# ricklisz/AnatoMask

Hardware: AMD Instinct MI355X
Metric: pretrain volumes/sec @128^3 patch mask=0.6 (higher is better)
Workload: dtype bf16; 1 GPU; STUNet-B AnatoMask step, 128^3 patch, mask_ratio 0.6, bf16 storage/MFMA + fp32 master; per_gpu_batch=16, global_batch=16, parallelism=dp1, step=teacher fwd + sampler + student fwd + loss + bwd + clip + AdamW + EMA

## Files before the change

### anatomask_amd/csrc/stream_ops.hip

```cpp
#include <mutex>
#include <type_traits>
#include "common.h"
#include "../../include/anatomask_hip.h"

namespace {

constexpr int NREP = 8;

struct Geo {
  int B, D, H, W, C;
  int vpw;
  unsigned mW, mH, mD;
  MaskView mask;
  __device__ __forceinline__ bool active(long v) const {
    if (!mask.m) return true;
    const unsigned u = (unsigned)v;
    const unsigned t1 = __umulhi(u, mW); const int w = u - t1 * W;
    const unsigned t2 = __umulhi(t1, mH); const int h = t1 - t2 * H;
    const unsigned b = __umulhi(t2, mD); const int d = t2 - b * D;
    return mask.active((int)b, d, h, w);
  }
  __device__ __forceinline__ void decode(long v, int& b, int& d, int& h, int& w) const {
    const unsigned u = (unsigned)v;
    const unsigned t1 = __umulhi(u, mW); w = u - t1 * W;
// ... 1223 lines not shown
#pragma unroll
      for (int i = 0; i < EPC; ++i) a1[i] += red[(vl * wk.cpv + threadIdx.x) * 8 + i];
#pragma unroll
    for (int i = 0; i < EPC; ++i) atomicAdd(&ar[threadIdx.x * EPC + i], a1[i]);
  }
  if (threadIdx.x == 0) atomicAdd(&ar[C], (double)redb[0] + (double)redb[1] + (double)redb[2] + (double)redb[3]);
  if (!last_workgroup(fin.ticket)) return;
  if (threadIdx.x == 0) {
    double t = 0.0;
    for (int r = 0; r < NREP; ++r) t += __longlong_as_double(atomicExch((unsigned long long*)&acc[(size_t)r * (C + 1) + C], 0ull));
    s0sh = t;
    fin.db[0] += (float)t;
  }
  __syncthreads();
  const double S0 = s0sh;
  for (int c = threadIdx.x; c < C; c += blockDim.x) {
    double S1 = 0.0;
    for (int r = 0; r < NREP; ++r) S1 += __longlong_as_double(atomicExch((unsigned long long*)&acc[(size_t)r * (C + 1) + c], 0ull));
    const double wc = fin.w[c], rs = fin.rstd[c];
    const double b1 = wc * S0, b2 = rs * wc * S1;
    const float gr = fin.gamma[c] * fin.rstd[c];
    fin.k0w[c] = gr * fin.w[c]; fin.k1[c] = gr * (float)(b1 / fin.n); fin.k2[c] = gr * (float)(b2 / fin.n);
    fin.dgamma[c] += (float)b2;
    fin.dbeta[c] += (float)b1;
    fin.dw[c] += (float)((double)fin.scale[c] * S1 + (double)fin.beta[c] * S0);
  }
  if (threadIdx.x == 0) atomicExch(fin.ticket, 0u);
}

template <typename T>
__global__ __launch_bounds__(256) void proj_norm_bwd_apply_kernel(const T* __restrict__ x, const float* __restrict__ drec, long nvox, int C,
                                                                  int vpw, const float* __restrict__ mean, const float* __restrict__ rstd,
                                                                  const float* __restrict__ k0w, const float* __restrict__ k1,
                                                                  const float* __restrict__ k2, T* __restrict__ dx) {
  constexpr int EPC = TT<T>::EPC;
  Walk<T> wk(C);
  if (!wk.live) return;
  float mu[EPC], c0[EPC], c1[EPC], c2[EPC];
#pragma unroll
  for (int i = 0; i < EPC; ++i) {
    const int c = wk.cl * EPC + i;
    mu[i] = mean[c]; c0[i] = k0w[c]; c1[i] = k1[c]; c2[i] = k2[c] * rstd[c];
  }
  const long v0 = (long)blockIdx.x * vpw, v1 = min(v0 + (long)vpw, nvox);
  for (long v = v0 + wk.vl; v < v1; v += wk.vpp) {
    const float d = drec[v];
    const size_t off = (size_t)v * C + wk.cl * EPC;
    float f[EPC], r[EPC];
    chunk_to_f<T>(*(const u32x4*)(x + off), f);
#pragma unroll
    for (int i = 0; i < EPC; ++i) r[i] = c0[i] * d - c1[i] - c2[i] * (f[i] - mu[i]);
    *(u32x4*)(dx + off) = f_to_chunk<T>(r);
  }
}

template <typename T>
__global__ __launch_bounds__(256) void proj_bwd_kernel(const T* __restrict__ x, const float* __restrict__ drec, long nvox, int C, int vpw,
                                                       const float* __restrict__ w, T* __restrict__ dx, float* __restrict__ dw,
                                                       float* __restrict__ db, float* __restrict__ det_ws) {
  constexpr int EPC = TT<T>::EPC;
  __shared__ float red[256 * 8];
  __shared__ float redb[4];
  Walk<T> wk(C);
  float sw[EPC], wv[EPC], sb = 0.f;
#pragma unroll
  for (int i = 0; i < EPC; ++i) { sw[i] = 0.f; wv[i] = wk.live ? w[wk.cl * EPC + i] : 0.f; }
  const long v0 = (long)blockIdx.x * vpw, v1 = min(v0 + (long)vpw, nvox);
  if (wk.live)
    for (long v = v0 + wk.vl; v < v1; v += wk.vpp) {
      const float d = drec[v];
      const size_t off = (size_t)v * C + wk.cl * EPC;
      float f[EPC], o[EPC];
      chunk_to_f<T>(*(const u32x4*)(x + off), f);
#pragma unroll
      for (int i = 0; i < EPC; ++i) { sw[i] += d * f[i]; o[i] = d * wv[i]; }
      *(u32x4*)(dx + off) = f_to_chunk<T>(o);
      if (wk.cl == 0) sb += d;
    }
#pragma unroll
  for (int i = 0; i < EPC; ++i) red[threadIdx.x * 8 + i] = sw[i];
  sb = warp_sum(sb);
  if ((threadIdx.x & 63) == 0) redb[threadIdx.x >> 6] = sb;
  __syncthreads();
  if (threadIdx.x < wk.cpv) {
    float a1[EPC];
#pragma unroll
// ... 590 lines not shown
}

int am_proj_fwd(int dtype, const void* x, long nvox, int C, const float* w, const float* b, const float* pre_scale, const float* pre_shift,
                float* rec, void* stream) {
  if (!am_row_ok(dtype, C, F32_MAX_C_256)) return -1;
  if ((pre_scale == nullptr) != (pre_shift == nullptr)) return -1;
  hipStream_t st = (hipStream_t)stream;
  const int nb = (int)((nvox + 255) / 256);
  am_by_dtype(dtype, [&](auto t) {
    using T = typename decltype(t)::type;
    AM_LAUNCH(proj_fwd_kernel<T>, dim3(nb), dim3(256), 0, st, (const T*)x, nvox, C, w, b, pre_scale, pre_shift, rec);
  });
  AM_CHECK_LAUNCH();
  return 0;
}

int am_proj_norm_bwd(int dtype, const void* x, const float* drec, long nvox, int C, const float* w, const float* gamma, const float* beta,
                     const float* mean, const float* rstd, const float* scale, double* workspace, float* coef, void* dx,
                     float* dgamma_accum, float* dbeta_accum, float* dw_accum, float* db_accum, void* stream) {
  if (!am_row_ok(dtype, C, F32_MAX_C_256)) return -1;
  if (!x || !drec || !w || !gamma || !beta || !mean || !rstd || !scale || !workspace || !coef || !dx || !dgamma_accum || !dbeta_accum ||
      !dw_accum || !db_accum || nvox <= 0) return -1;
  hipStream_t st = (hipStream_t)stream;
  ProjNormFin fin{(unsigned*)(workspace + (size_t)NREP * (C + 1)), (double)nvox, gamma, beta, rstd, scale, w,
                  coef, coef + C, coef + 2 * C, dgamma_accum, dbeta_accum, dw_accum, db_accum};
  const int vr = pick_vpw(nvox, C, dtype, true), va = pick_vpw(nvox, C, dtype, false);
  am_by_dtype(dtype, [&](auto t) {
    using T = typename decltype(t)::type;
    AM_LAUNCH(proj_norm_bwd_reduce_kernel<T>, dim3(nblk(nvox, vr)), dim3(256), 0, st, (const T*)x, drec, nvox, C, vr, mean, workspace, fin);
  });
  AM_CHECK_LAUNCH();
  am_by_dtype(dtype, [&](auto t) {
    using T = typename decltype(t)::type;
    AM_LAUNCH(proj_norm_bwd_apply_kernel<T>, dim3(nblk(nvox, va)), dim3(256), 0, st, (const T*)x, drec, nvox, C, va, mean, rstd, coef, coef + C, coef + 2 * C, (T*)dx);
  });
  AM_CHECK_LAUNCH();
  return 0;
}

int am_proj_bwd(int dtype, const void* x, const float* drec, long nvox, int C, const float* w, void* dx, float* dw_accum,
                float* db_accum, float* det_workspace, long det_workspace_floats, void* stream) {
  if (!am_row_ok(dtype, C, F32_MAX_C_256)) return -1;
  hipStream_t st = (hipStream_t)stream;
  const int vpw = pick_vpw(nvox, C, dtype, true);
  const int nb = nblk(nvox, vpw);
  if (det_workspace && det_workspace_floats < (long)nb * (C + 1)) return -6;
  am_by_dtype(dtype, [&](auto t) {
    using T = typename decltype(t)::type;
    AM_LAUNCH(proj_bwd_kernel<T>, dim3(nb), dim3(256), 0, st, (const T*)x, drec, nvox, C, vpw, w, (T*)dx, dw_accum, db_accum, det_workspace);
  });
  AM_CHECK_LAUNCH();
  if (det_workspace) {
    AM_LAUNCH(rows_fold_kernel, dim3((C + 1 + 255) / 256), dim3(256), 0, st, det_workspace, nb, C + 1, C, dw_accum, db_accum);
    AM_CHECK_LAUNCH();
  }
  return 0;
}

int am_partials_reduce(const float* partials, int rows, int C, double* sums, float* sum_accum, void* stream) {
  hipStream_t st = (hipStream_t)stream;
  if ((256 % C == 0 || C % 256 == 0) && rows >= 64) {
    const int rstep = C <= 256 ? 256 / C : 1;
    int nb = rows / (rstep * 16); nb = nb < 1 ? 1 : (nb > 256 ? 256 : nb);
    const int rpb = ((rows + nb - 1) / nb + rstep - 1) / rstep * rstep;
    nb = (rows + rpb - 1) / rpb;
    if (sums) AM_HIP(hipMemsetAsync(sums, 0, sizeof(double) * 2 * C, st));
    AM_LAUNCH(partials_reduce2_kernel, dim3(nb), dim3(256), 0, st, partials, rows, C, rpb, sums, sum_accum);
// ... 83 lines not shown
```

### anatomask_amd/engine.py

```python
from __future__ import annotations

from dataclasses import dataclass, field
from typing import Dict, List, Optional, Sequence, Tuple

import torch

from . import ops
from .ops import ACT_LRELU, ACT_NONE, ACT_RELU6, CONV_DGRAD, CONV_FWD, CONVT_DGRAD, CONVT_FWD, MaskInfo, NormStats

ENC = "sparse_encoder.sp_cnn.conv_blocks_context"
DEC = "dense_decoder.dec"


@dataclass
class Spec:
    dims: Sequence[int]
    depth: Sequence[int]
    width: int
    input_size: Tuple[int, int, int]
    in_ch: int = 1
    out_ch: int = 1
    downsample: int = 16
    n_stage: int = 5
    sync_bn: bool = False
# ... 261 lines not shown
    x = None
    for s in range(spec.n_stage):
        sp = spec.stage_spatial(s)
        if tape is not None and recompute:
            tape.enc_in.append(x)
        for b in range(spec.depth[s]):
            x, rec_ = _enc_block(W, pk, inp, mask, counts, sp, s, b, x, keep=tape is not None)
            if tape is not None and not recompute:
                tape.enc.append(rec_)
        feats.append(x)
    return feats


def densify_forward(spec: Spec, W, pk: PackCache, feats, mask: MaskInfo, counts, tape: Optional[Tape] = None) -> List[torch.Tensor]:
    n_dec = len(spec.dec_chs) - 1
    to_dec = []
    for i in range(n_dec):
        f = feats[4 - i]
        st = _sparse_norm(f, mask, i, counts, W[f"densify_norms.{i}.weight"], W[f"densify_norms.{i}.bias"], 1e-6)
        d = ops.norm_apply(f, st, ACT_NONE, mask, i, fill=W[f"mask_tokens.{i}"].view(-1))
        pw = f"densify_projs.{i}.weight"
        if pw in W:
            k = W[pw].shape[-1]
            pr = ops.conv3d(CONV_FWD, d, pk.get(W, pw, False, False), W[f"densify_projs.{i}.bias"], tuple(d.shape[1:4]), k, 1)
        else:
            pr = d
        to_dec.append(pr)
        if tape is not None:
            tape.dens.append({"i": i, "f": f, "st": st, "d": d, "k": W[pw].shape[-1] if pw in W else 0})
    return to_dec


HEAD_STENCIL = True


def decoder_forward(spec: Spec, W, pk: PackCache, to_dec, train: bool, tape: Optional[Tape] = None, recompute: bool = False,
                    needed_patches: Optional[MaskInfo] = None, fuse_eval: Optional[bool] = None, l2_of: Optional[tuple] = None) -> torch.Tensor:
    n_dec = len(spec.dec_chs) - 1
    if fuse_eval is None:
        fuse_eval = tape is None
    x = to_dec[0]
    head = bool(train and FUSED_HEAD and _sync_world(spec.sync_bn) <= 1 and not spec.dec_inorm)
    st_head = None
    for i in range(n_dec):
        nxt = to_dec[i + 1] if i + 1 < n_dec else None
        last = i == n_dec - 1
        o, rec_ = _dec_block(W, pk, i, x, nxt, train, fuse_eval=fuse_eval,
                             out_skip=needed_patches if (last and tape is None and not train) else None, sync=spec.sync_bn,
                             head=head and last, inorm=spec.dec_inorm,
                             stencil_tail=bool(HEAD_STENCIL and last and tape is None and not train and fuse_eval and not spec.dec_inorm))
        if rec_ is not None and rec_.get("stencil"):
            q = f"{DEC}.{i}"
            weff, beff = ops.head_fold(W[f"{q}.conv.3.weight"], rec_["st2"].scale, rec_["st2"].shift, W["dense_decoder.proj.weight"].view(-1),
                                       W["dense_decoder.proj.bias"])
            B_, D_, H_, W_ = o.shape[:4]
            patches = needed_patches
            if patches is None:
                patches = MaskInfo(torch.ones(B_, D_ // 16, H_ // 16, W_ // 16, device=o.device, dtype=torch.uint8), n_active=B_ * (D_ // 16) * (H_ // 16) * (W_ // 16))
            if l2_of is not None:
                ops.head_stencil(o, weff, beff, patches, inp=l2_of[0], l2=l2_of[1])
                return None
            rec = torch.empty(B_, D_, H_, W_, device=o.device, dtype=torch.float32)
            ops.head_stencil(o, weff, beff, patches, rec=rec)
            return rec
        if head and last:
            st_head = rec_["st2"]
        if tape is not None:
            tape.dec.append({"q": rec_["q"], "xin": x, "nxt": nxt, "head": head and last} if recompute else rec_)
        x = o
    rec = ops.proj_fwd(x, W["dense_decoder.proj.weight"].view(-1), W["dense_decoder.proj.bias"], pre=st_head)
    if tape is not None:
        tape.last = x
    return rec


def forward(spec: Spec, W: Dict[str, torch.Tensor], pk: PackCache, inp: torch.Tensor, mask: MaskInfo, train: bool,
            tape: Optional[Tape] = None, want_feats: bool = False, encoder_only: bool = False, recompute: bool = False,
            want_to_dec0: bool = False, needed_patches: Optional[MaskInfo] = None, l2_out: Optional[torch.Tensor] = None):
    counts = _counts(mask, range(5))
    if tape is not None:
        tape.counts = counts
        tape.recompute = recompute
    feats = encoder_forward(spec, W, pk, inp, mask, counts, tape, recompute)
    if encoder_only:
        return feats
    to_dec = densify_forward(spec, W, pk, feats, mask, counts, tape)
    rec = decoder_forward(spec, W, pk, to_dec, train, tape, recompute, needed_patches, l2_of=(inp, l2_out) if l2_out is not None else None)
    if want_to_dec0:
        return rec, to_dec[0]
    return (rec, feats) if want_feats else rec


FUSED_HEAD = True
_SIDE: Dict[int, "torch.cuda.Stream"] = {}
_SIDE_KEEP: Dict[int, List[torch.Tensor]] = {}
_USE_SIDE = True


def _dev_index(dev) -> int:
    return dev.index if dev.index is not None else torch.cuda.current_device()


def _side_stream(dev) -> "torch.cuda.Stream":
    i = _dev_index(dev)
    if i not in _SIDE:
        _SIDE[i] = torch.cuda.Stream(device=dev)
    return _SIDE[i]


def _on_side(dev, tensors, fn):
    if not _USE_SIDE:
        return fn()
    s2 = _side_stream(dev)
    ev = torch.cuda.Event()
    ev.record()
    s2.wait_event(ev)
    _SIDE_KEEP.setdefault(_dev_index(dev), []).extend(tensors)
    with torch.cuda.stream(s2):
        fn()


def _join_side(dev):
    i = _dev_index(dev)
    if _USE_SIDE and i in _SIDE:
        ev = torch.cuda.Event()
        ev.record(_SIDE[i])
        torch.cuda.current_stream(dev).wait_event(ev)
    _SIDE_KEEP.pop(i, None)


def _wgrad_into(pk: PackCache, G, name, mode, x, dy, k, stride, transposed=False, **masks):
    def run():
        dwp = ops.conv3d_wgrad(mode, x, dy, k, stride, f32_split=pk.f32_split, deterministic=pk.deterministic, **masks)
        ops.unpack_grad(dwp, G[name], transposed, accumulate=True)
    _on_side(x.device, (x, dy), run)


def _dec_block_backward(W, G, pk: PackCache, t: dict, g: Optional[torch.Tensor], drec: Optional[torch.Tensor], bias_sum_into: Optional[torch.Tensor]):
    q = t["q"]
    if t.get("inorm"):
        so = tuple(t["r"].shape[1:4])
        dc2 = _instance_norm_backward(g, t["c2"], t["st2"], ACT_NONE)
        dr = ops.conv3d(CONV_DGRAD, dc2, pk.get(W, f"{q}.conv.3.weight", False, True), None, so, 3, 1)
        _wgrad_into(pk, G, f"{q}.conv.3.weight", CONV_FWD, t["r"], dc2, 3, 1)
        dc1 = _instance_norm_backward(dr, t["c1"], t["st1"], ACT_RELU6)
    elif t.get("head"):
        dc2 = ops.proj_norm_bwd(t["c2"], t["st2"], drec, W["dense_decoder.proj.weight"].view(-1), W[f"{q}.conv.4.weight"],
                                W[f"{q}.conv.4.bias"], G[f"{q}.conv.4.weight"], G[f"{q}.conv.4.bias"],
                                G["dense_decoder.proj.weight"].view(-1), G["dense_decoder.proj.bias"])
    else:
        dc2 = ops.norm_backward(g, None, t["c2"], t["st2"], W[f"{q}.conv.4.weight"], ACT_NONE, None, 0,
                                G[f"{q}.conv.4.weight"], G[f"{q}.conv.4.bias"])
    if not t.get("inorm"):
        so = tuple(t["r"].shape[1:4])
        fuse = ops.FUSED_NORM_BWD_REDUCE and dc2.dtype == torch.bfloat16 and t["st1"].sync_world <= 1 and dc2.shape[-1] >= 128
        dr = ops.conv3d(CONV_DGRAD, dc2, pk.get(W, f"{q}.conv.3.weight", False, True), None, so, 3, 1,
                        norm_bwd=(t["c1"], t["st1"], ACT_RELU6) if fuse else None)
        dr, red1 = dr if fuse else (dr, None)
        _wgrad_into(pk, G, f"{q}.conv.3.weight", CONV_FWD, t["r"], dc2, 3, 1)
        dc1 = ops.norm_backward(dr, None, t["c1"], t["st1"], W[f"{q}.conv.1.weight"], ACT_RELU6, None, 0,
                                G[f"{q}.conv.1.weight"], G[f"{q}.conv.1.bias"], reduced=red1)
    du, ptu = ops.conv3d(CONV_DGRAD, dc1, pk.get(W, f"{q}.conv.0.weight", False, True), None, so, 3, 1, want_partials=True, partials_sum_only=True)
    ptu.finalize(None, sum_accum=G[f"{q}.up_sample.bias"])
    _wgrad_into(pk, G, f"{q}.conv.0.weight", CONV_FWD, t["u"], dc1, 3, 1)
    si = tuple(t["xin"].shape[1:4])
    gin = ops.conv3d(CONVT_DGRAD, du, pk.get(W, f"{q}.up_sample.weight", True, True), None, si, 4, 2, want_partials=bias_sum_into is not None)
    if bias_sum_into is not None:
        gin, ptg = gin
        ptg.finalize(None, sum_accum=bias_sum_into)
    _wgrad_into(pk, G, f"{q}.up_sample.weight", CONVT_FWD, t["xin"], du, 4, 2, transposed=True)
    return gin


def decoder_backward(spec: Spec, W, G, pk: PackCache, tape: Tape, drec: torch.Tensor, after_group=None) -> List[Optional[torch.Tensor]]:
    n_dec = len(spec.dec_chs) - 1
    fused_head = bool(tape.dec[n_dec - 1].get("head"))
    g = None
    if not fused_head:
# ... 175 lines not shown
```

### anatomask_amd/hip.py

```python
import ctypes as C
import os
import re

_HERE = os.path.dirname(os.path.abspath(__file__))
LIB_PATH = os.path.join(_HERE, "libanatomask_hip.so")
HEADER = os.path.join(os.path.dirname(_HERE), "include", "anatomask_hip.h")

DT_F32, DT_BF16, DT_F32S = 0, 1, 2
CONV_FWD, CONV_DGRAD, CONVT_FWD, CONVT_DGRAD = 0, 1, 2, 3
ACT_NONE, ACT_LRELU, ACT_RELU6 = 0, 1, 2

_CT = {"int": C.c_int, "long": C.c_long, "float": C.c_float, "double": C.c_double}


def declared_functions(header: str = HEADER):
    txt = open(header).read()
    txt = re.sub(r"/\*.*?\*/", " ", txt, flags=re.S)
    out = {}
    for m in re.finditer(r"\bint\s+(am_\w+)\s*\(([^;]*?)\)\s*;", txt, flags=re.S):
        name, args = m.group(1), m.group(2).strip()
        types = []
        if args and args != "void":
            for a in args.split(","):
                a = " ".join(a.split())
                if "*" in a:
                    types.append(C.c_void_p)
                else:
                    types.append(_CT[a.replace("const ", "").split(" ")[0]])
        out[name] = types
    return out


class HipLib:
    ANSWERS = ("am_head_stencil_supported", "am_conv3d_wgrad_uses_k3", "am_conv3d_uses_k3", "am_conv3d_prenorm_supported", "am_version")

    def __init__(self, path: str = LIB_PATH):
        import torch
        if not os.path.exists(path):
            raise RuntimeError(f"{path} not built: run `python -m anatomask_amd.build` (no fallback path exists)")
        if os.path.abspath(path) == LIB_PATH:
            from . import build as _b
            sp = _b.stamp_path(path)
            have = open(sp).read().strip() if os.path.exists(sp) else None
            if have != _b.source_digest():
                raise RuntimeError(f"{path} was not built from the csrc/ + include/ sources next to it (stamp {str(have)[:12]}.. != sources "
                                   f"{_b.source_digest()[:12]}..): run `python -m anatomask_amd.build`")
        self._lib = C.CDLL(path)
        self.functions = declared_functions()
        for name, argtypes in self.functions.items():
            fn = getattr(self._lib, name)
            fn.argtypes = argtypes
            fn.restype = C.c_int
            if name not in self.ANSWERS:
                setattr(self, name[3:], self._wrap(name, fn))

    @staticmethod
    def _wrap(name, fn):
        def call(*args):
            rc = fn(*args)
            if rc != 0:
                raise RuntimeError(f"{name} failed with code {rc}")
        call.__name__ = name
        return call


_LIB = None

# ... 15 lines not shown
```

### anatomask_amd/ops.py

```python
from __future__ import annotations

from typing import Optional, Tuple

import torch

from . import hip
from .hip import ACT_LRELU, ACT_NONE, ACT_RELU6, CONV_DGRAD, CONV_FWD, CONVT_DGRAD, CONVT_FWD


def _dt(t: torch.Tensor) -> int:
    if t.dtype == torch.float32:
        return hip.DT_F32
    if t.dtype == torch.bfloat16:
        return hip.DT_BF16
    raise TypeError(f"unsupported dtype {t.dtype}")


DEFAULT_F32_SPLIT = False


def _dtc(t: torch.Tensor, f32_split: bool) -> int:
    return hip.DT_F32S if (t.dtype == torch.float32 and f32_split) else _dt(t)


# ... 466 lines not shown
    B, D, H, W, Cc = x.shape
    mp, fd, fh, fw = _mk(mask)
    hip.lib().chan_sum(_dt(x), x.data_ptr(), B, D, H, W, Cc, mp, bshift, fd, fh, fw, out_accum.data_ptr(), _stream())


def add(a: torch.Tensor, b: torch.Tensor, out: Optional[torch.Tensor] = None) -> torch.Tensor:
    if out is None:
        out = torch.empty_like(a)
    hip.lib().add(_dt(a), a.data_ptr(), b.data_ptr(), out.data_ptr(), a.numel(), _stream())
    return out


def proj_fwd(x: torch.Tensor, w: torch.Tensor, b: torch.Tensor, pre: Optional["NormStats"] = None) -> torch.Tensor:
    B, D, H, W, Cc = x.shape
    rec = torch.empty(B, D, H, W, device=x.device, dtype=torch.float32)
    hip.lib().proj_fwd(_dt(x), x.data_ptr(), B * D * H * W, Cc, w.data_ptr(), b.data_ptr(), _p(pre.scale) if pre else None,
                       _p(pre.shift) if pre else None, rec.data_ptr(), _stream())
    return rec


def proj_norm_bwd(x: torch.Tensor, st: "NormStats", drec: torch.Tensor, w: torch.Tensor, gamma: torch.Tensor, beta: torch.Tensor,
                  dgamma: torch.Tensor, dbeta: torch.Tensor, dw_accum: torch.Tensor, db_accum: torch.Tensor) -> torch.Tensor:
    B, D, H, W, Cc = x.shape
    assert st.sync_world <= 1
    dx = torch.empty_like(x)
    ws_b, _ = _bwd_workspaces(x.device, Cc)
    coef = torch.empty(3, Cc, device=x.device, dtype=torch.float32)
    hip.lib().proj_norm_bwd(_dt(x), x.data_ptr(), drec.data_ptr(), B * D * H * W, Cc, w.data_ptr(), gamma.data_ptr(), beta.data_ptr(),
                            st.mean.data_ptr(), st.rstd.data_ptr(), st.scale.data_ptr(), ws_b.data_ptr(), coef.data_ptr(), dx.data_ptr(),
                            dgamma.data_ptr(), dbeta.data_ptr(), dw_accum.data_ptr(), db_accum.data_ptr(), _stream())
    return dx


def proj_bwd(x: torch.Tensor, drec: torch.Tensor, w: torch.Tensor, dw_accum: torch.Tensor, db_accum: torch.Tensor,
             deterministic: Optional[bool] = None) -> torch.Tensor:
    B, D, H, W, Cc = x.shape
    dx = torch.empty_like(x)
    ws = _det_workspace(x.device, 4096 * (Cc + 1) // 8) if _det(deterministic) else None
    hip.lib().proj_bwd(_dt(x), x.data_ptr(), drec.data_ptr(), B * D * H * W, Cc, w.data_ptr(), dx.data_ptr(), dw_accum.data_ptr(),
                       db_accum.data_ptr(), _p(ws), ws.numel() if ws is not None else 0, _stream())
    return dx


def head_stencil_supported(x: torch.Tensor) -> bool:
    B, D, H, W, C = x.shape
    ok = hip.lib()._lib.am_head_stencil_supported(_dt(x), C) == 1
    return bool(ok and D % 16 == 0 and H % 16 == 0 and W % 16 == 0 and max(B, D // 16, H // 16, W // 16) <= 255)


def head_fold(w2: torch.Tensor, scale: torch.Tensor, shift: torch.Tensor, wproj: torch.Tensor, bproj: torch.Tensor):
    cmid, cin = w2.shape[0], w2.shape[1]
    assert tuple(w2.shape[2:]) == (3, 3, 3) and w2.is_contiguous() and wproj.numel() == cmid
    weff = torch.empty(27, cin, device=w2.device, dtype=torch.float32)
    beff = torch.empty(1, device=w2.device, dtype=torch.float32)
    hip.lib().head_fold(w2.data_ptr(), cmid, cin, scale.data_ptr(), shift.data_ptr(), wproj.data_ptr(), bproj.data_ptr(), weff.data_ptr(),
                        beff.data_ptr(), _stream())
    return weff, beff


def head_stencil(r: torch.Tensor, weff: torch.Tensor, beff: torch.Tensor, patches: MaskInfo, rec: Optional[torch.Tensor] = None,
                 inp: Optional[torch.Tensor] = None, l2: Optional[torch.Tensor] = None):
    B, D, H, W, C = r.shape
    lst, n = patches.active_list()
    assert lst is not None and (patches.fd, patches.fh, patches.fw) == (D // 16, H // 16, W // 16) and r.is_contiguous()
    assert rec is None or (rec.dtype == torch.float32 and tuple(rec.shape) == (B, D, H, W) and rec.is_contiguous())
    assert l2 is None or (inp is not None and l2.dtype == torch.float32 and l2.numel() == B * patches.fd * patches.fh * patches.fw)
# ... 170 lines not shown
```

### anatomask_amd/trainer.py

```python
from __future__ import annotations

from typing import Dict, Optional

import torch
import torch.distributed as dist

from . import engine, ops
from .modules import ModelEma, SparK, ema_decay_for_epoch


class _Range:
    __slots__ = ("on",)

    def __init__(self, on: bool, name: str):
        self.on = on
        if on:
            torch.cuda.nvtx.range_push(name)

    def __enter__(self):
        return self

    def __exit__(self, *exc):
        if self.on:
            torch.cuda.nvtx.range_pop()
# ... 214 lines not shown
             keys: Optional[torch.Tensor] = None, lr: Optional[float] = None, ema_decay: Optional[float] = None):
        m, t = self.model, self.teacher.ema
        spec = m.spec
        x = inp_bchwd[:, 0].float().contiguous()
        B = x.shape[0]
        L = spec.fmap[0] * spec.fmap[1] * spec.fmap[2]
        dev = x.device
        if mask1 is None:
            k1 = torch.rand(B, L, device=dev, generator=self.gen)
            m1 = ops.mask_sampler(torch.zeros(B, L, device=dev), k1, m.len_keep, 0)
        else:
            m1 = mask1.reshape(B, L).to(device=dev, dtype=torch.uint8).contiguous()
        mi1 = ops.MaskInfo(m1.view(B, *spec.fmap), n_active=B * m.len_keep if mask1 is None else None)
        tr_ = self.trace_ranges
        if self.self_distill:
            with _Range(tr_, "anatomask.teacher_forward"):
                need = ops.MaskInfo((1 - m1).view(B, *spec.fmap), n_active=B * (L - m.len_keep) if mask1 is None else None) if spec.input_size[0] // spec.fmap[0] == 16 else None
                recon = torch.zeros(B, L, device=dev) if need is not None else None
                rec1 = engine.forward(spec, t._W, t._pack, x, mi1, train=False, needed_patches=need, l2_out=recon)
                if rec1 is not None:
                    recon, _, _, _ = ops.patch_loss_fwd(x, rec1, mi1, normalized=False, want_loss=False)
                del rec1
            with _Range(tr_, "anatomask.mask_sampler"):
                ll = m.len_loss_for(L, m.len_keep, epoch, self.total_epochs - 1, self.guide)
                if keys is None:
                    keys = torch.rand(B, L, device=dev, generator=self.gen)
                mk = ops.mask_sampler(recon, keys.to(dev).float().contiguous(), m.len_keep, ll)
                mi = ops.MaskInfo(mk.view(B, *spec.fmap), n_active=B * m.len_keep)
        else:
            recon, mk, mi = None, m1, mi1
        self._snap_b.copy_(m._bflat); self._snap_i.copy_(m._iflat)
        tape = engine.Tape()
        with _Range(tr_, "anatomask.student_forward"):
            rec = engine.forward(spec, m._W, m._pack, x, mi, train=True, tape=tape, recompute=m.recompute)
            l2m, pm, pr, info = ops.patch_loss_fwd(x, rec, mi, normalized=True)
            drec = ops.patch_loss_bwd(x, rec, mi, pm, pr, info, None)
        with _Range(tr_, "anatomask.backward"):
            m._gflat.zero_()
            if self.distributed and not self._capturing:
                self._exchange_begin()
            engine.backward(spec, m._W, m._G, m._pack, x, mi, tape, drec, self._after_group if self.distributed else None, join_before_hook=False)
            del tape
        with _Range(tr_, "anatomask.exchange_wait"):
            self._finish_exchange()
        rng_opt = _Range(tr_, "anatomask.optimizer_ema")
        n = m._live_end
        decay = self.teacher.decay if ema_decay is None else ema_decay
        ops.sumsq(m._gflat[:n], self.sumsq)
        dyn = None
        if self._capturing:
            dyn = self._dyn_dev
        else:
            self.step_count += 1
        ops.adamw_ema(m._flat, m._gflat, self.m, self.v, t._flat if self.self_distill else None, n, self.lr if lr is None else lr,
                      self.betas, self.eps, self.wd, max(self.step_count, 1), self.sumsq, self.clip, decay, self.gnorm,
                      grad_scale=self.grad_scale, dyn=dyn, guard=self.guard)
        ops.guard_restore(m._bflat, self._snap_b, self.guard)
        ops.guard_restore(m._iflat, self._snap_i, self.guard)
        if not self.self_distill:
            m.weights_changed()
            rng_opt.__exit__()
            return {"loss": info[0:1], "grad_norm": self.gnorm, "mask": mk, "recon_loss": None, "rec_loss": l2m}
        if m._flat.numel() > n:
            ops.ema(t._flat[n:], m._flat[n:], decay, self.guard)
        ops.ema(t._bflat, m._bflat, decay, self.guard)
        if m._n_ibuf:
            ops.ema_i64(t._iflat[:m._n_ibuf], m._iflat[:m._n_ibuf], decay, self.guard)
        m.weights_changed(); t.weights_changed()
        rng_opt.__exit__()
        return {"loss": info[0:1], "grad_norm": self.gnorm, "mask": mk, "recon_loss": recon, "rec_loss": l2m}

# ... 64 lines not shown
```

### include/anatomask_hip.h

```cpp
#ifndef ANATOMASK_HIP_H
#define ANATOMASK_HIP_H
#include <stdint.h>
#ifdef __cplusplus
extern "C" {
#endif

#define AM_DT_F32 0
#define AM_DT_BF16 1
#define AM_DT_F32S 2

#define AM_CONV_PARTIALS_SUM_ONLY 2
#define AM_CONV_FWD 0
#define AM_CONV_DGRAD 1
#define AM_CONVT_FWD 2
#define AM_CONVT_DGRAD 3

#define AM_DXREP 64
#define AM_NREP 8

#define AM_ACT_NONE 0
#define AM_ACT_LRELU 1
#define AM_ACT_RELU6 2

int am_version(void);
// ... 90 lines not shown
                       const float* pre_scale, const float* pre_shift ,
                       const int32_t* active_list, int n_active,
                       const double* count_ptr, double count_host, const float* gamma, float* k0, float* k1, float* k2,
                       float* dgamma_accum, float* dbeta_accum, float* dtoken_accum, float* dbeta2_accum
                       ,
                       void* stream);
int am_norm_bwd_finalize(const double* bsum, const double* count_ptr, double count_host, int C, const float* gamma,
                         const float* rstd, float* k0, float* k1, float* k2, float* dgamma_accum, float* dbeta_accum,
                         float* dtoken_accum, float* dbeta2_accum , void* stream);
int am_norm_bwd_apply(int dtype, const void* dout, const void* out, const void* x, int B, int D, int H, int W, int C,
                      const uint8_t* mask, int bshift, int fd, int fh, int fw, const float* mean, const float* rstd,
                      const float* k0, const float* k1, const float* k2, int act, void* dx, void* dres,
                      float* dxsum_accum ,
                      double* dxsum_scratch ,
                      const float* pre_scale, const float* pre_shift ,
                      const int32_t* active_list, int n_active,
                      int scratch_is_zero_workspace , void* stream);
int am_chan_sum(int dtype, const void* x, int B, int D, int H, int W, int C, const uint8_t* mask, int bshift, int fd, int fh,
                int fw, float* out_accum, void* stream);
int am_add(int dtype, const void* a, const void* b, void* y, long n_elems, void* stream);

int am_head_fold(const float* w2, int cmid, int cin, const float* scale, const float* shift, const float* wproj, const float* bproj,
                 float* weff, float* beff, void* stream);
int am_head_stencil(int dtype, const void* r, int B, int D, int H, int W, int C, const float* weff, const float* beff,
                    const int32_t* patch_list, int n_patches, float* rec , const float* inp ,
                    float* l2 , void* stream);
int am_head_stencil_supported(int dtype, int C);

int am_proj_fwd(int dtype, const void* x, long nvox, int C, const float* w, const float* b,
                const float* pre_scale, const float* pre_shift , float* rec, void* stream);
int am_proj_norm_bwd(int dtype, const void* x, const float* drec, long nvox, int C, const float* w, const float* gamma, const float* beta,
                     const float* mean, const float* rstd, const float* scale, double* workspace, float* coef, void* dx,
                     float* dgamma_accum, float* dbeta_accum, float* dw_accum, float* db_accum, void* stream);
int am_proj_bwd(int dtype, const void* x, const float* drec, long nvox, int C, const float* w, void* dx, float* dw_accum,
                float* db_accum, float* det_workspace, long det_workspace_floats , void* stream);

int am_patch_loss_fwd(const float* inp, const float* rec, const uint8_t* active, int B, int D, int H, int W, int normalized,
                      float* l2m, float* pmean, float* prstd, float* lossinfo, void* stream);
int am_patch_loss_bwd(const float* inp, const float* rec, const uint8_t* active, int B, int D, int H, int W, const float* pmean,
                      const float* prstd, const float* lossinfo, const float* gout, float* drec, void* stream);

int am_mask_sampler(const float* loss, const float* keys, int B, int L, int len_keep, int len_loss, uint8_t* mask, void* stream);

int am_sumsq(const float* g, long n, double* out, void* stream);
int am_adamw_ema(float* p, const float* g, float* m, float* v, float* ema , long n, double lr, double beta1,
                 double beta2, double eps, double weight_decay, int step, const double* sumsq ,
                 double max_norm, double ema_decay, double grad_scale ,
                 float* gnorm_out,
                 const float* dyn_scalars ,
                 int* guard ,
                 void* stream);
int am_ema(float* ema, const float* p, long n, double decay, const int* guard , void* stream);
int am_ema_i64(long* ema, const long* p, int n, double decay, const int* guard, void* stream);
int am_guard_restore(void* dst, const void* snapshot, long nbytes, const int* guard, void* stream);

int am_spline_prefilter(float* vol, int D, int H, int W, void* stream);
int am_resample_affine(const float* src, int Ds, int Hs, int Ws, float* dst, int D, int H, int W, const float* affine_host12, int order,
                       float cval, void* stream);


#define AM_LAYER_REP 64
int am_voxel_norm_fwd(int dtype, int kind, const void* x, void* y, int B, int D, int H, int W, int C, int groups, const float* gamma,
                      const float* beta, float eps, const uint8_t* mask, int bshift, const int32_t* active_list, int n_active, void* stream);
int am_voxel_norm_bwd(int dtype, int kind, const void* x, const void* dy, void* dx, int B, int D, int H, int W, int C, int groups,
                      const float* gamma, float eps, float* dgamma_accum, float* dbeta_accum, const uint8_t* mask, int bshift,
                      const int32_t* active_list, int n_active, void* stream);
// ... 49 lines not shown
```

Baseline: 140.4 volumes/s.

## Fuse decoder head projection, patch loss and norm-backward reduction into one kernel

Adds a head_loss kernel that, per 16^3 patch, normalizes the input target, computes the 1x1 projection of the normed decoder output, forms the residual, and accumulates the loss plus the projection/instance-norm backward reductions in a single pass. The last workgroup finalizes the loss scalars and norm-backward coefficients. The apply kernel then scales the stored residual by a device-side factor. This replaces separate proj_fwd, patch_loss_fwd, patch_loss_bwd and proj_norm_bwd reduce passes, cutting several full-volume reads of the decoder activations and the reconstruction. It only applies in non-deterministic mode and when shapes and channel counts fit, and the zeroing of the gradient buffer moves before the forward pass.

```diff
diff --git a/anatomask_amd/csrc/stream_ops.hip b/anatomask_amd/csrc/stream_ops.hip
--- a/anatomask_amd/csrc/stream_ops.hip
+++ b/anatomask_amd/csrc/stream_ops.hip
@@ -1279,10 +1279,12 @@
 __global__ __launch_bounds__(256) void proj_norm_bwd_apply_kernel(const T* __restrict__ x, const float* __restrict__ drec, long nvox, int C,
                                                                   int vpw, const float* __restrict__ mean, const float* __restrict__ rstd,
                                                                   const float* __restrict__ k0w, const float* __restrict__ k1,
-                                                                  const float* __restrict__ k2, T* __restrict__ dx) {
+                                                                  const float* __restrict__ k2, const float* __restrict__ kptr,
+                                                                  T* __restrict__ dx) {
   constexpr int EPC = TT<T>::EPC;
   Walk<T> wk(C);
   if (!wk.live) return;
+  const float kk = kptr ? kptr[0] : 1.f;
   float mu[EPC], c0[EPC], c1[EPC], c2[EPC];
 #pragma unroll
   for (int i = 0; i < EPC; ++i) {
@@ -1291,7 +1293,7 @@
   }
   const long v0 = (long)blockIdx.x * vpw, v1 = min(v0 + (long)vpw, nvox);
   for (long v = v0 + wk.vl; v < v1; v += wk.vpp) {
-    const float d = drec[v];
+    const float d = kptr ? kk * drec[v] : drec[v];
     const size_t off = (size_t)v * C + wk.cl * EPC;
     float f[EPC], r[EPC];
     chunk_to_f<T>(*(const u32x4*)(x + off), f);
@@ -1299,6 +1301,159 @@
     for (int i = 0; i < EPC; ++i) r[i] = c0[i] * d - c1[i] - c2[i] * (f[i] - mu[i]);
     *(u32x4*)(dx + off) = f_to_chunk<T>(r);
   }
+}
+
+template <typename T>
+__global__ __launch_bounds__(256) void head_loss_kernel(const T* __restrict__ x, const float* __restrict__ inp, const uint8_t* __restrict__ active,
+                                                        int D, int H, int W, int fd, int fh, int fw, int C, int normalized,
+                                                        const float* __restrict__ mean, const float* __restrict__ psc,
+                                                        const float* __restrict__ psh, const float* __restrict__ w,
+                                                        const float* __restrict__ b, const float* __restrict__ gout,
+                                                        float* __restrict__ e_out, float* __restrict__ l2m, float* __restrict__ info,
+                                                        double* __restrict__ acc, ProjNormFin fin) {
+  constexpr int EPC = TT<T>::EPC;
+  __shared__ __attribute__((aligned(16))) double fold[256 * 8];
+  float* tgt = (float*)fold;
+  __shared__ float sh[4], redb[4], redl[4];
+  __shared__ double s0sh;
+  __shared__ float ksh;
+  const int L = fd * fh * fw;
+  const int bb = blockIdx.x / L, l = blockIdx.x % L;
+  const int pw = l % fw, ph = (l / fw) % fh, pd = l / (fw * fh);
+  const size_t pbase = (((size_t)bb * D + pd * 16) * H + ph * 16) * W + pw * 16;
+  if (active[blockIdx.x]) {
+    const size_t base = pbase + ((size_t)(threadIdx.x >> 4) * H + (threadIdx.x & 15)) * W;
+#pragma unroll
+    for (int q = 0; q < 4; ++q) *(f32x4*)(e_out + base + 4 * q) = f32x4{0.f, 0.f, 0.f, 0.f};
+    if (threadIdx.x == 0) l2m[blockIdx.x] = 0.f;
+  } else {
+    {
+      const size_t base = pbase + ((size_t)(threadIdx.x >> 4) * H + (threadIdx.x & 15)) * W;
+      float xi[16];
+#pragma unroll
+      for (int q = 0; q < 4; ++q) {
+        const f32x4 a = *(const f32x4*)(inp + base + 4 * q);
+#pragma unroll
+        for (int i = 0; i < 4; ++i) xi[4 * q + i] = a[i];
+      }
+      float pm = 0.f, pr = 1.f;
+      if (normalized) {
+        float s = 0.f;
+#pragma unroll
+        for (int i = 0; i < 16; ++i) s += xi[i];
+        s = warp_sum(s);
+        if ((threadIdx.x & 63) == 0) sh[threadIdx.x >> 6] = s;
+        __syncthreads();
+        pm = (sh[0] + sh[1] + sh[2] + sh[3]) * (1.f / 4096.f);
+        float s2 = 0.f;
+#pragma unroll
+        for (int i = 0; i < 16; ++i) { const float d = xi[i] - pm; s2 += d * d; }
+        s2 = warp_sum(s2);
+        __syncthreads();
+        if ((threadIdx.x & 63) == 0) sh[threadIdx.x >> 6] = s2;
+        __syncthreads();
+        pr = 1.f / sqrtf((sh[0] + sh[1] + sh[2] + sh[3]) * (1.f / 4095.f) + 1e-6f);
+      }
+#pragma unroll
+      for (int i = 0; i < 16; ++i) tgt[threadIdx.x * 16 + i] = (xi[i] - pm) * pr;
+    }
+    __syncthreads();
+    Walk<T> wk(C);
+    float s1[EPC], mu[EPC], sc[EPC], sf[EPC], wv[EPC], sb = 0.f, l2 = 0.f;
+    double d1[EPC];
+#pragma unroll
+    for (int i = 0; i < EPC; ++i) {
+      const int c = wk.cl * EPC + i;
+      s1[i] = 0.f; d1[i] = 0.0; mu[i] = mean[c]; sc[i] = psc[c]; sf[i] = psh[c]; wv[i] = w[c];
+    }
+    const float bias = b[0];
+    const int np = 4096 / wk.vpp;
+    for (int it = 0; it < np; it += 4) {
+      if (it && (it & 15) == 0) {
+#pragma unroll
+        for (int i = 0; i < EPC; ++i) { d1[i] += (double)s1[i]; s1[i] = 0.f; }
+      }
+      u32x4 cv[4]; size_t vo[4]; int pv[4];
+#pragma unroll
+      for (int u = 0; u < 4; ++u) {
+        const int p = (it + u) * wk.vpp + wk.vl;
+        pv[u] = p;
+        vo[u] = pbase + ((size_t)(p >> 8) * H + ((p >> 4) & 15)) * W + (p & 15);
+        cv[u] = *(const u32x4*)(x + vo[u] * C + wk.cl * EPC);
+      }
+#pragma unroll
+      for (int u = 0; u < 4; ++u) {
+        float f[EPC];
+        chunk_to_f<T>(cv[u], f);
+        float part = 0.f;
+#pragma unroll
+        for (int i = 0; i < EPC; ++i) part += (f[i] * sc[i] + sf[i]) * wv[i];
+        for (int o = wk.cpv >> 1; o > 0; o >>= 1) part += __shfl_xor(part, o, 64);
+        const float e = bias + part - tgt[pv[u]];
+#pragma unroll
+        for (int i = 0; i < EPC; ++i) s1[i] += e * (f[i] - mu[i]);
+        if (wk.cl == 0) { sb += e; l2 += e * e; e_out[vo[u]] = e; }
+      }
+    }
+    __syncthreads();
+#pragma unroll
+    for (int i = 0; i < EPC; ++i) fold[threadIdx.x * 8 + i] = d1[i] + (double)s1[i];
+    sb = warp_sum(sb); l2 = warp_sum(l2);
+    if ((threadIdx.x & 63) == 0) { redb[threadIdx.x >> 6] = sb; redl[threadIdx.x >> 6] = l2; }
+    __syncthreads();
+    double* ar = acc + (size_t)(blockIdx.x % NREP) * (C + 2);
+    if (threadIdx.x < wk.cpv) {
+      double a1[EPC];
+#pragma unroll
+      for (int i = 0; i < EPC; ++i) a1[i] = 0.0;
+      for (int vl = 0; vl < wk.vpp; ++vl)
+#pragma unroll
+        for (int i = 0; i < EPC; ++i) a1[i] += fold[(vl * wk.cpv + threadIdx.x) * 8 + i];
+#pragma unroll
+      for (int i = 0; i < EPC; ++i) atomicAdd(&ar[threadIdx.x * EPC + i], a1[i]);
+    }
+    if (threadIdx.x == 0) {
+      const float pl = (redl[0] + redl[1] + redl[2] + redl[3]) * (1.f / 4096.f);
+      l2m[blockIdx.x] = pl;
+      atomicAdd(&ar[C], (double)redb[0] + (double)redb[1] + (double)redb[2] + (double)redb[3]);
+      atomicAdd(&ar[C + 1], (double)pl);
+    }
+  }
+  if (!last_workgroup(fin.ticket)) return;
+  float cnt = 0.f;
+  for (int i = threadIdx.x; i < (int)gridDim.x; i += 256) cnt += active[i] ? 0.f : 1.f;
+  cnt = warp_sum(cnt);
+  if ((threadIdx.x & 63) == 0) sh[threadIdx.x >> 6] = cnt;
+  __syncthreads();
+  if (threadIdx.x == 0) {
+    cnt = sh[0] + sh[1] + sh[2] + sh[3];
+    double t = 0.0, ls = 0.0;
+    for (int r = 0; r < NREP; ++r) {
+      t += __longlong_as_double(atomicExch((unsigned long long*)&acc[(size_t)r * (C + 2) + C], 0ull));
+      ls += __longlong_as_double(atomicExch((unsigned long long*)&acc[(size_t)r * (C + 2) + C + 1], 0ull));
+    }
+    const float lossv = (float)ls / (cnt + 1e-8f), inv = 1.f / (cnt + 1e-8f);
+    const float k = lossv - lossv == 0.f ? (gout ? gout[0] : 1.f) * inv * (2.f / 4096.f) : __builtin_nanf("");
+    info[0] = lossv; info[1] = inv; info[2] = k;
+    ksh = k;
+    s0sh = (double)k * t;
+    fin.db[0] += (float)s0sh;
+  }
+  __syncthreads();
+  const double S0 = s0sh, kd = (double)ksh;
+  for (int c = threadIdx.x; c < C; c += blockDim.x) {
+    double S1 = 0.0;
+    for (int r = 0; r < NREP; ++r) S1 += __longlong_as_double(atomicExch((unsigned long long*)&acc[(size_t)r * (C + 2) + c], 0ull));
+    S1 *= kd;
+    const double wc = fin.w[c], rs = fin.rstd[c];
+    const double b1 = wc * S0, b2 = rs * wc * S1;
+    const float gr = fin.gamma[c] * fin.rstd[c];
+    fin.k0w[c] = gr * fin.w[c]; fin.k1[c] = gr * (float)(b1 / fin.n); fin.k2[c] = gr * (float)(b2 / fin.n);
+    fin.dgamma[c] += (float)b2;
+    fin.dbeta[c] += (float)b1;
+    fin.dw[c] += (float)((double)fin.scale[c] * S1 + (double)fin.beta[c] * S0);
+  }
+  if (threadIdx.x == 0) atomicExch(fin.ticket, 0u);
 }
 
 template <typename T>
@@ -1955,7 +2110,48 @@
   AM_CHECK_LAUNCH();
   am_by_dtype(dtype, [&](auto t) {
     using T = typename decltype(t)::type;
-    AM_LAUNCH(proj_norm_bwd_apply_kernel<T>, dim3(nblk(nvox, va)), dim3(256), 0, st, (const T*)x, drec, nvox, C, va, mean, rstd, coef, coef + C, coef + 2 * C, (T*)dx);
+    AM_LAUNCH(proj_norm_bwd_apply_kernel<T>, dim3(nblk(nvox, va)), dim3(256), 0, st, (const T*)x, drec, nvox, C, va, mean, rstd, coef, coef + C, coef + 2 * C, (const float*)nullptr, (T*)dx);
+  });
+  AM_CHECK_LAUNCH();
+  return 0;
+}
+
+int am_head_loss_supported(int dtype, int C) {
+  if (!am_row_ok(dtype, C, F32_MAX_C_256)) return 0;
+  const int cpv = C / (dtype == AM_DT_BF16 ? 8 : 4);
+  return cpv <= 64 && (cpv & (cpv - 1)) == 0;
+}
+
+int am_head_loss(int dtype, const void* x, const float* inp, const uint8_t* active, int B, int D, int H, int W, int C, int normalized,
+                 const float* w, const float* b, const float* gamma, const float* beta, const float* mean, const float* rstd,
+                 const float* scale, const float* shift, const float* gout, double* workspace, float* coef, float* e, float* l2m,
+                 float* info, float* dgamma_accum, float* dbeta_accum, float* dw_accum, float* db_accum, void* stream) {
+  if (!am_head_loss_supported(dtype, C)) return -1;
+  if (!x || !inp || !active || !w || !b || !gamma || !beta || !mean || !rstd || !scale || !shift || !workspace || !coef || !e || !l2m ||
+      !info || !dgamma_accum || !dbeta_accum || !dw_accum || !db_accum) return -1;
+  if (B <= 0 || D <= 0 || H <= 0 || W <= 0 || D % 16 || H % 16 || W % 16) return -1;
+  const int fd = D / 16, fh = H / 16, fw = W / 16;
+  if ((long)B * fd * fh * fw > 0x7fffffffL) return -4;
+  const long nvox = (long)B * D * H * W;
+  ProjNormFin fin{(unsigned*)(workspace + (size_t)NREP * (C + 2)), (double)nvox, gamma, beta, rstd, scale, w,
+                  coef, coef + C, coef + 2 * C, dgamma_accum, dbeta_accum, dw_accum, db_accum};
+  am_by_dtype(dtype, [&](auto t) {
+    using T = typename decltype(t)::type;
+    AM_LAUNCH(head_loss_kernel<T>, dim3(B * fd * fh * fw), dim3(256), 0, (hipStream_t)stream, (const T*)x, inp, active, D, H, W, fd, fh, fw, C,
+              normalized, mean, scale, shift, w, b, gout, e, l2m, info, workspace, fin);
+  });
+  AM_CHECK_LAUNCH();
+  return 0;
+}
+
+int am_proj_norm_bwd_apply(int dtype, const void* x, const float* e, const float* k, long nvox, int C, const float* mean, const float* rstd,
+                           const float* coef, void* dx, void* stream) {
+  if (!am_row_ok(dtype, C, F32_MAX_C_256)) return -1;
+  if (!x || !e || !k || !mean || !rstd || !coef || !dx || nvox <= 0) return -1;
+  const int va = pick_vpw(nvox, C, dtype, false);
+  am_by_dtype(dtype, [&](auto t) {
+    using T = typename decltype(t)::type;
+    AM_LAUNCH(proj_norm_bwd_apply_kernel<T>, dim3(nblk(nvox, va)), dim3(256), 0, (hipStream_t)stream, (const T*)x, e, nvox, C, va, mean, rstd, coef, coef + C, coef + 2 * C, k, (T*)dx);
   });
   AM_CHECK_LAUNCH();
   return 0;
diff --git a/anatomask_amd/engine.py b/anatomask_amd/engine.py
--- a/anatomask_amd/engine.py
+++ b/anatomask_amd/engine.py
@@ -317,10 +317,24 @@
 
 
 HEAD_STENCIL = True
+FUSED_HEAD_LOSS = True
+
+
+class LossRequest:
+
+    def __init__(self, inp: torch.Tensor, mask: MaskInfo, normalized: bool, G: Dict[str, torch.Tensor], gout: Optional[torch.Tensor] = None):
+        self.inp, self.mask, self.normalized, self.G, self.gout = inp, mask, normalized, G, gout
+        self.out = None
+
+    def serves(self, x: torch.Tensor) -> bool:
+        B, D, H, W = x.shape[:4]
+        m = self.mask
+        return bool(tuple(self.inp.shape) == (B, D, H, W) and (m.fd * 16, m.fh * 16, m.fw * 16) == (D, H, W) and ops.head_loss_supported(x))
 
 
 def decoder_forward(spec: Spec, W, pk: PackCache, to_dec, train: bool, tape: Optional[Tape] = None, recompute: bool = False,
-                    needed_patches: Optional[MaskInfo] = None, fuse_eval: Optional[bool] = None, l2_of: Optional[tuple] = None) -> torch.Tensor:
+                    needed_patches: Optional[MaskInfo] = None, fuse_eval: Optional[bool] = None, l2_of: Optional[tuple] = None,
+                    loss: Optional["LossRequest"] = None) -> torch.Tensor:
     n_dec = len(spec.dec_chs) - 1
     if fuse_eval is None:
         fuse_eval = tape is None
@@ -353,6 +367,15 @@
         if tape is not None:
             tape.dec.append({"q": rec_["q"], "xin": x, "nxt": nxt, "head": head and last} if recompute else rec_)
         x = o
+    if (st_head is not None and loss is not None and FUSED_HEAD_LOSS and tape is not None and not recompute
+            and not (pk.deterministic or ops.DETERMINISTIC_WGRAD) and loss.serves(x)):
+        q, G = f"{DEC}.{n_dec - 1}", loss.G
+        loss.out = ops.head_loss(x, st_head, W["dense_decoder.proj.weight"].view(-1), W["dense_decoder.proj.bias"], W[f"{q}.conv.4.weight"],
+                                 W[f"{q}.conv.4.bias"], loss.inp, loss.mask, loss.normalized, loss.gout, G[f"{q}.conv.4.weight"],
+                                 G[f"{q}.conv.4.bias"], G["dense_decoder.proj.weight"].view(-1), G["dense_decoder.proj.bias"])
+        tape.dec[n_dec - 1]["head_loss"] = loss.out
+        tape.last = x
+        return None
     rec = ops.proj_fwd(x, W["dense_decoder.proj.weight"].view(-1), W["dense_decoder.proj.bias"], pre=st_head)
     if tape is not None:
         tape.last = x
@@ -361,7 +384,8 @@
 
 def forward(spec: Spec, W: Dict[str, torch.Tensor], pk: PackCache, inp: torch.Tensor, mask: MaskInfo, train: bool,
             tape: Optional[Tape] = None, want_feats: bool = False, encoder_only: bool = False, recompute: bool = False,
-            want_to_dec0: bool = False, needed_patches: Optional[MaskInfo] = None, l2_out: Optional[torch.Tensor] = None):
+            want_to_dec0: bool = False, needed_patches: Optional[MaskInfo] = None, l2_out: Optional[torch.Tensor] = None,
+            loss: Optional["LossRequest"] = None):
     counts = _counts(mask, range(5))
     if tape is not None:
         tape.counts = counts
@@ -370,7 +394,8 @@
     if encoder_only:
         return feats
     to_dec = densify_forward(spec, W, pk, feats, mask, counts, tape)
-    rec = decoder_forward(spec, W, pk, to_dec, train, tape, recompute, needed_patches, l2_of=(inp, l2_out) if l2_out is not None else None)
+    rec = decoder_forward(spec, W, pk, to_dec, train, tape, recompute, needed_patches, l2_of=(inp, l2_out) if l2_out is not None else None,
+                          loss=loss)
     if want_to_dec0:
         return rec, to_dec[0]
     return (rec, feats) if want_feats else rec
@@ -429,6 +454,8 @@
         dr = ops.conv3d(CONV_DGRAD, dc2, pk.get(W, f"{q}.conv.3.weight", False, True), None, so, 3, 1)
         _wgrad_into(pk, G, f"{q}.conv.3.weight", CONV_FWD, t["r"], dc2, 3, 1)
         dc1 = _instance_norm_backward(dr, t["c1"], t["st1"], ACT_RELU6)
+    elif t.get("head") and drec is None:
+        dc2 = ops.proj_norm_bwd_apply(t["c2"], t["st2"], t["head_loss"])
     elif t.get("head"):
         dc2 = ops.proj_norm_bwd(t["c2"], t["st2"], drec, W["dense_decoder.proj.weight"].view(-1), W[f"{q}.conv.4.weight"],
                                 W[f"{q}.conv.4.bias"], G[f"{q}.conv.4.weight"], G[f"{q}.conv.4.bias"],
diff --git a/anatomask_amd/hip.py b/anatomask_amd/hip.py
--- a/anatomask_amd/hip.py
+++ b/anatomask_amd/hip.py
@@ -32,7 +32,7 @@
 
 
 class HipLib:
-    ANSWERS = ("am_head_stencil_supported", "am_conv3d_wgrad_uses_k3", "am_conv3d_uses_k3", "am_conv3d_prenorm_supported", "am_version")
+    ANSWERS = ("am_head_stencil_supported", "am_head_loss_supported", "am_conv3d_wgrad_uses_k3", "am_conv3d_uses_k3", "am_conv3d_prenorm_supported", "am_version")
 
     def __init__(self, path: str = LIB_PATH):
         import torch
diff --git a/anatomask_amd/ops.py b/anatomask_amd/ops.py
--- a/anatomask_amd/ops.py
+++ b/anatomask_amd/ops.py
@@ -522,6 +522,45 @@
     return dx
 
 
+def head_loss_supported(x: torch.Tensor) -> bool:
+    B, D, H, W, Cc = x.shape
+    return bool(hip.lib()._lib.am_head_loss_supported(_dt(x), Cc) == 1 and D % 16 == 0 and H % 16 == 0 and W % 16 == 0)
+
+
+class HeadLoss:
+    __slots__ = ("e", "k", "coef", "l2m", "info")
+
+    def __init__(self, e, k, coef, l2m, info):
+        self.e, self.k, self.coef, self.l2m, self.info = e, k, coef, l2m, info
+
+
+def head_loss(x: torch.Tensor, st: "NormStats", w: torch.Tensor, b: torch.Tensor, gamma: torch.Tensor, beta: torch.Tensor,
+              inp: torch.Tensor, mask: MaskInfo, normalized: bool, gout: Optional[torch.Tensor], dgamma: torch.Tensor,
+              dbeta: torch.Tensor, dw_accum: torch.Tensor, db_accum: torch.Tensor) -> HeadLoss:
+    B, D, H, W, Cc = x.shape
+    assert st.sync_world <= 1 and tuple(inp.shape) == (B, D, H, W) and inp.dtype == torch.float32 and inp.is_contiguous()
+    assert (mask.fd, mask.fh, mask.fw) == (D // 16, H // 16, W // 16) and x.is_contiguous()
+    L = mask.fd * mask.fh * mask.fw
+    e = torch.empty(B, D, H, W, device=x.device, dtype=torch.float32)
+    l2m = torch.empty(B, L, device=x.device, dtype=torch.float32)
+    info = torch.empty(3, device=x.device, dtype=torch.float32)
+    coef = torch.empty(3, Cc, device=x.device, dtype=torch.float32)
+    ws_b, _ = _bwd_workspaces(x.device, Cc)
+    hip.lib().head_loss(_dt(x), x.data_ptr(), inp.data_ptr(), mask.t.data_ptr(), B, D, H, W, Cc, int(normalized), w.data_ptr(), b.data_ptr(),
+                        gamma.data_ptr(), beta.data_ptr(), st.mean.data_ptr(), st.rstd.data_ptr(), st.scale.data_ptr(), st.shift.data_ptr(),
+                        _p(gout), ws_b.data_ptr(), coef.data_ptr(), e.data_ptr(), l2m.data_ptr(), info.data_ptr(), dgamma.data_ptr(),
+                        dbeta.data_ptr(), dw_accum.data_ptr(), db_accum.data_ptr(), _stream())
+    return HeadLoss(e, info[2:3], coef, l2m, info)
+
+
+def proj_norm_bwd_apply(x: torch.Tensor, st: "NormStats", hl: HeadLoss) -> torch.Tensor:
+    B, D, H, W, Cc = x.shape
+    dx = torch.empty_like(x)
+    hip.lib().proj_norm_bwd_apply(_dt(x), x.data_ptr(), hl.e.data_ptr(), hl.k.data_ptr(), B * D * H * W, Cc, st.mean.data_ptr(),
+                                  st.rstd.data_ptr(), hl.coef.data_ptr(), dx.data_ptr(), _stream())
+    return dx
+
+
 def proj_bwd(x: torch.Tensor, drec: torch.Tensor, w: torch.Tensor, dw_accum: torch.Tensor, db_accum: torch.Tensor,
              deterministic: Optional[bool] = None) -> torch.Tensor:
     B, D, H, W, Cc = x.shape
diff --git a/anatomask_amd/trainer.py b/anatomask_amd/trainer.py
--- a/anatomask_amd/trainer.py
+++ b/anatomask_amd/trainer.py
@@ -270,11 +270,16 @@
         self._snap_b.copy_(m._bflat); self._snap_i.copy_(m._iflat)
         tape = engine.Tape()
         with _Range(tr_, "anatomask.student_forward"):
-            rec = engine.forward(spec, m._W, m._pack, x, mi, train=True, tape=tape, recompute=m.recompute)
-            l2m, pm, pr, info = ops.patch_loss_fwd(x, rec, mi, normalized=True)
-            drec = ops.patch_loss_bwd(x, rec, mi, pm, pr, info, None)
+            m._gflat.zero_()
+            req = engine.LossRequest(x, mi, True, m._G)
+            rec = engine.forward(spec, m._W, m._pack, x, mi, train=True, tape=tape, recompute=m.recompute, loss=req)
+            if req.out is not None:
+                l2m, info, drec = req.out.l2m, req.out.info, None
+            else:
+                l2m, pm, pr, info = ops.patch_loss_fwd(x, rec, mi, normalized=True)
+                drec = ops.patch_loss_bwd(x, rec, mi, pm, pr, info, None)
+            del rec
         with _Range(tr_, "anatomask.backward"):
-            m._gflat.zero_()
             if self.distributed and not self._capturing:
                 self._exchange_begin()
             engine.backward(spec, m._W, m._G, m._pack, x, mi, tape, drec, self._after_group if self.distributed else None, join_before_hook=False)
diff --git a/include/anatomask_hip.h b/include/anatomask_hip.h
--- a/include/anatomask_hip.h
+++ b/include/anatomask_hip.h
@@ -146,6 +146,13 @@
 int am_proj_norm_bwd(int dtype, const void* x, const float* drec, long nvox, int C, const float* w, const float* gamma, const float* beta,
                      const float* mean, const float* rstd, const float* scale, double* workspace, float* coef, void* dx,
                      float* dgamma_accum, float* dbeta_accum, float* dw_accum, float* db_accum, void* stream);
+int am_head_loss(int dtype, const void* x, const float* inp, const uint8_t* active, int B, int D, int H, int W, int C, int normalized,
+                 const float* w, const float* b, const float* gamma, const float* beta, const float* mean, const float* rstd,
+                 const float* scale, const float* shift, const float* gout , double* workspace, float* coef, float* e,
+                 float* l2m, float* info, float* dgamma_accum, float* dbeta_accum, float* dw_accum, float* db_accum, void* stream);
+int am_head_loss_supported(int dtype, int C);
+int am_proj_norm_bwd_apply(int dtype, const void* x, const float* e, const float* k, long nvox, int C, const float* mean, const float* rstd,
+                           const float* coef, void* dx, void* stream);
 int am_proj_bwd(int dtype, const void* x, const float* drec, long nvox, int C, const float* w, void* dx, float* dw_accum,
                 float* db_accum, float* det_workspace, long det_workspace_floats , void* stream);
 
```

Result: no change. 141.2 volumes/s, median of 6 (+0.6%).
